# redhat-et/aws-k8s-ansible-provisioner

Measured on AMD Instinct MI355X. Metric: output tok/s + p50 TTFT, higher is better.
Workload: dtype bf16

## Files before the change

aws_k8s_ansible_provisioner_amd/csrc/kernels/kernels.h:

```cpp
#pragma once

#include <hip/hip_runtime.h>
#include <stdint.h>

#include "host_contract.h"

namespace akap {

void launch_rmsnorm(void* out, const void* x, const void* w, int rows, int d, int x_stride,
                    int out_stride, float eps, hipStream_t s);
void launch_fused_add_rmsnorm(void* out, void* residual, const void* x, const void* w, int rows,
                              int d, int x_stride, int out_stride, float eps, hipStream_t s);

void launch_qk_norm_rope_cache(const void* qkv, int qkv_stride, void* q_out, void* k_cache,
                               void* v_cache, const int64_t* positions, const int64_t* slots,
                               const float* cos_sin, const void* q_w, const void* k_w, int T,
                               int Hq, int Hkv, int D, int BS, float eps, int apply_rope,
                               hipStream_t s, int kv_fp8 = 0, int v_per_token = 0,
                               void* v_tail = nullptr, const int* tail_slot = nullptr,
                               int num_decode = 0, int q_rows = -1);
void launch_reshape_and_cache(const void* k, const void* v, void* k_cache, void* v_cache,
                              const int64_t* slots, int T, int Hkv, int D, int BS, hipStream_t s,
                              int kv_fp8 = 0);

// ... 131 lines not shown
void launch_moe_combine_split(const float* P, const float* wts, const int32_t* inv, void* out,
                              int T, int topk, int d, int S, int rows, hipStream_t s);

void launch_moe_topk_softmax(const void* logits, int ld, int E, int K, float* topk_w,
                             int32_t* topk_ids, int T, int renormalize, hipStream_t s);
void launch_moe_router_topk(const void* h, int ldh, const void* W, int d, int E, int K,
                            float* topk_w, int32_t* topk_ids, int T, int renormalize,
                            hipStream_t s);
void launch_moe_align(const int32_t* topk_ids, int n, int E, int block, int32_t* sorted_ids,
                      int32_t* expert_offsets, int32_t* num_padded, int32_t* inv,
                      int32_t* tile_expert, int max_tiles, hipStream_t s);
void launch_moe_gemm(const void* A, const void* W, void* Y, const int32_t* sorted_ids,
                     const int32_t* tile_expert, int max_tiles, int n_flat, int topk, int N,
                     int K, int lda, int gather, hipStream_t s);
void launch_moe_combine(const void* Y, const float* wts, const int32_t* inv, void* out, int T,
                        int topk, int d, hipStream_t s);

void launch_kv_gather(const void* cache, long plane_stride, int planes, int block_elems,
                      int cache_blocks, const int* block_ids, int nblk, void* out,
                      hipStream_t s);
void launch_kv_scatter(const void* in, void* cache, long plane_stride, int planes,
                       int block_elems, int cache_blocks, const int* block_ids, int nblk,
                       hipStream_t s);
struct KVPullArgs {
  const int64_t* src_planes;
  const int64_t* dst_planes;
  int planes, block_elems;
  const int* pairs;
  int nblk;
  __bf16* tail;
  const int* tail_jobs;
  int ntail, layers, tail_slots, Hkv, BS, D;
};
void launch_kv_pull(const KVPullArgs& a, hipStream_t s);

void launch_embedding_prep(const int64_t* ids, const void* table, const void* ln, void* residual,
                           void* a_out, float* ss_out, float* zbuf, long zn, int T, int d,
                           int vocab_start, int vocab_end, hipStream_t s);
void launch_embedding(const int64_t* ids, const void* table, void* out, int T, int d,
                      int vocab_start, int vocab_end, hipStream_t s);

struct CarArgs {
  __bf16* bufs[8];
  uint32_t* sigs[8];
  uint32_t* counter;
  uint32_t* err;
  int rank, world;
  size_t half_elems;
  int blocks;
};
struct CarEpi {
  __bf16* residual;
  const __bf16* ln;
  __bf16* aout;
  float* ss;
  int d;
};
void launch_custom_allreduce(const CarArgs& a, const void* in, void* out, long n, int two_shot,
                             hipStream_t s, const CarEpi* epi = nullptr);
size_t custom_allreduce_signal_bytes();
void launch_custom_allgather(const CarArgs& a, const void* in, void* out, long rows, int n,
                             hipStream_t s);
void launch_custom_broadcast(const CarArgs& a, void* buf, long bytes, int root, hipStream_t s);
void launch_custom_alltoall(const CarArgs& a, const void* in, void* out, long seg_elems,
                            hipStream_t s);
struct CarMulti {
  CarArgs args[8];
  const void* in[8];
  void* out[8];
  CarEpi epi[8];
  int use_epi;
  int warm;
};
void launch_custom_allreduce_multi(const CarMulti& m, int world, long n, int two_shot,
                                   hipStream_t s);

struct PrefetchList {
  const void* ptr[8];
  long bytes[8];
  int n;
};
void launch_l2_prefetch(const PrefetchList& L, uint32_t* sink, hipStream_t s);
void launch_h2d_stage(const void* host_src, void* dst, long bytes, hipStream_t s);

}
```

aws_k8s_ansible_provisioner_amd/csrc/kernels/prefetch.hip:

```cpp
#include "common.h"
#include "kernels.h"

namespace akap {

__global__ __launch_bounds__(256) void l2_prefetch_kernel(PrefetchList L, uint32_t* sink) {
  uint32_t acc = 0;
  const long gid = (long)blockIdx.x * 256 + threadIdx.x;
  const long stride = (long)gridDim.x * 256;
  for (int i = 0; i < L.n; ++i) {
    const u32x4* p = reinterpret_cast<const u32x4*>(L.ptr[i]);
    const long n16 = L.bytes[i] >> 4;
    for (long j = gid; j < n16; j += stride) acc ^= p[j].x;
  }
  if (acc == 0x9E3779B9u && gid == 0) sink[0] = acc;
}

void launch_l2_prefetch(const PrefetchList& L, uint32_t* sink, hipStream_t s) {
  long total = 0;
  for (int i = 0; i < L.n; ++i) total += L.bytes[i];
  if (total == 0) return;
  long blocks = (total / 16 + 255) / 256;
  if (blocks > 2048) blocks = 2048;
  l2_prefetch_kernel<<<(int)blocks, 256, 0, s>>>(L, sink);
}

__global__ __launch_bounds__(256) void h2d_stage_kernel(const uint8_t* __restrict__ src,
                                                        uint8_t* __restrict__ dst, long bytes) {
  const long gid = (long)blockIdx.x * 256 + threadIdx.x;
  const long stride = (long)gridDim.x * 256;
  const long n16 = bytes >> 4;
  for (long j = gid; j < n16; j += stride)
    reinterpret_cast<u32x4*>(dst)[j] = __builtin_nontemporal_load(reinterpret_cast<const u32x4*>(src) + j);
  for (long j = (n16 << 4) + gid; j < bytes; j += stride) dst[j] = src[j];
}

void launch_h2d_stage(const void* host_src, void* dst, long bytes, hipStream_t s) {
  if (bytes <= 0) return;
  long blocks = ((bytes >> 4) + 255) / 256;
  if (blocks < 1) blocks = 1;
  if (blocks > 64) blocks = 64;
  h2d_stage_kernel<<<(int)blocks, 256, 0, s>>>((const uint8_t*)host_src, (uint8_t*)dst, bytes);
}

}
```

aws_k8s_ansible_provisioner_amd/csrc/kernels/wgemm.hip:

```cpp
#include <cstdlib>

#include "gemm_common.h"

namespace akap {

constexpr int WNS = 3;

template <int WM>
struct WCfg {
  static constexpr int BM = 64 * WM;
  static constexpr int WN = 8 / WM;
  static constexpr int BN = WM == 4 ? 128 : 256;
  static constexpr int WC = BN / WN;
  static constexpr int JN = WC / 16;
  static constexpr int GA = WM;
  static constexpr int GW = BN / 64;
  static constexpr int G = GA + GW;
  static constexpr int SU = (BM + BN) * 8;
  static constexpr int EP = WC + 8;
};

template <int WM, bool NTW = false>
__global__ __launch_bounds__(512, 2) void wgemm_kernel(WGemmArgs p) {
  using C = WCfg<WM>;
// ... 117 lines not shown
  const bf16* X = static_cast<const bf16*>(p.X);
  const bf16* W = static_cast<const bf16*>(p.W);
  const int lr = lane >> 2;
  const int lc = (lane & 3) ^ ((0x1320 >> (4 * ((lr >> 2) & 3))) & 3);
  const bf16* asrc[GA];
  const bf16* wsrc[GW];
#pragma unroll
  for (int i = 0; i < GA; ++i) {
    const int row = (w * GA + i) * 16 + lr;
    asrc[i] = X + (size_t)(row < p.M ? row : 0) * p.ldx + lc * 8;
  }
#pragma unroll
  for (int i = 0; i < GW; ++i) {
    const int v = n0 + (w * GW + i) * 16 + lr;
    wsrc[i] = W + (size_t)(v < p.N ? v : 0) * p.ldw + lc * 8;
  }
  auto issue = [&](int step) {
    bf16x8* slot = lds + (step % NS) * SU;
    const int k0 = step * BK;
#pragma unroll
    for (int i = 0; i < GA; ++i) glds16(asrc[i] + k0, slot + (w * GA + i) * 64);
#pragma unroll
    for (int i = 0; i < GW; ++i)
      glds16<NTW ? kAuxNT : 0>(wsrc[i] + k0, slot + BM * 4 + (w * GW + i) * 64);
  };

  f32x4 acc[4][JN];
#pragma unroll
  for (int i = 0; i < 4; ++i)
#pragma unroll
    for (int j = 0; j < JN; ++j) acc[i][j] = f32x4{0.f, 0.f, 0.f, 0.f};

#pragma unroll
  for (int s = 0; s < NS - 1; ++s)
    if (s < nk) issue(s);
  for (int t = 0; t < nk; ++t) {
    if (t + 2 < nk) wait_vm<2 * G>();
    else if (t + 1 < nk) wait_vm<G>();
    else asm volatile("s_waitcnt vmcnt(0)" ::: "memory");
    asm volatile("s_waitcnt lgkmcnt(0)" ::: "memory");
    __builtin_amdgcn_s_barrier();
    if (t + NS - 1 < nk) issue(t + NS - 1);
    const bf16x8* slot = lds + (t % NS) * SU;
    bf16x8 af[4], bfr[JN];
#pragma unroll
    for (int i = 0; i < 4; ++i) af[i] = slot[ww_swz(wm * 64 + i * 16 + fr, fg)];
#pragma unroll
    for (int j = 0; j < JN; ++j) bfr[j] = slot[BM * 4 + ww_swz(wn * WC + j * 16 + fr, fg)];
#pragma unroll
    for (int i = 0; i < 4; ++i)
#pragma unroll
      for (int j = 0; j < JN; ++j)
        acc[i][j] = __builtin_amdgcn_mfma_f32_16x16x32_bf16(af[i], bfr[j], acc[i][j], 0, 0, 0);
  }

  asm volatile("s_waitcnt lgkmcnt(0)" ::: "memory");
  __builtin_amdgcn_s_barrier();
  bf16* et = reinterpret_cast<bf16*>(lds) + (size_t)w * 64 * EP;
#pragma unroll
  for (int i = 0; i < 4; ++i)
#pragma unroll
    for (int j = 0; j < JN; ++j)
#pragma unroll
      for (int r = 0; r < 4; ++r) et[(i * 16 + fg * 4 + r) * EP + j * 16 + fr] = f2bf(acc[i][j][r]);
  asm volatile("s_waitcnt lgkmcnt(0)" ::: "memory");
  bf16* Y = static_cast<bf16*>(p.Y);
  constexpr int CPR = WC / 8;
  for (int e = lane; e < 64 * CPR; e += 64) {
    const int rr = e / CPR, cc = e % CPR;
    const int row = wm * 64 + rr;
    const int col = n0 + wn * WC + cc * 8;
    if (row >= p.M || col >= p.N) continue;
    const bf16* src = et + rr * EP + cc * 8;
    bf16* dst = Y + (size_t)row * p.ldy + col;
    if (col + 8 <= p.N) {
      bf16x8 v;
#pragma unroll
      for (int q = 0; q < 8; ++q) v[q] = src[q];
      *reinterpret_cast<bf16x8*>(dst) = v;
    } else {
      for (int q = 0; q < p.N - col; ++q) dst[q] = src[q];
    }
  }
}

static int wgemm_wide() {
  static const int v = [] {
    const char* e = std::getenv("AKAP_WGEMM_WIDE");
    return e ? std::atoi(e) : 0;
  }();
  return v;
}

int wgemm_rows(int M) { return M <= 64 ? 1 : (M <= 128 ? 2 : 4); }

void launch_wgemm(const WGemmArgs& p, hipStream_t st) {
  if (p.M == 0 || p.N == 0) return;
  const int wmr = wgemm_rows(p.M);
  const int bm = 64 * wmr, bn = wmr == 4 ? 128 : 256;
  dim3 grid((p.N + bn - 1) / bn, (p.M + bm - 1) / bm);
  static const bool nt = [] {
    const char* e = std::getenv("AKAP_WGEMM_NT");
    return e == nullptr || std::atoi(e) != 0;
  }();
  if (wmr == 4 && p.M <= 256 && wgemm_wide() == 1 && p.K % 32 == 0) {
    const dim3 gw((p.N + 255) / 256);
    if (nt) wgemm_wide_kernel<true><<<gw, 512, 0, st>>>(p);
    else wgemm_wide_kernel<false><<<gw, 512, 0, st>>>(p);
    return;
  }
  switch (wmr) {
    case 1: if (nt) wgemm_kernel<1, true><<<grid, 512, 0, st>>>(p); else wgemm_kernel<1><<<grid, 512, 0, st>>>(p); break;
    case 2: if (nt) wgemm_kernel<2, true><<<grid, 512, 0, st>>>(p); else wgemm_kernel<2><<<grid, 512, 0, st>>>(p); break;
    default: if (nt) wgemm_kernel<4, true><<<grid, 512, 0, st>>>(p); else wgemm_kernel<4><<<grid, 512, 0, st>>>(p); break;
  }
}

}
```

aws_k8s_ansible_provisioner_amd/csrc/ops.cpp:

```cpp
#include <algorithm>
#include <cstdlib>
#include <cstring>
#include <vector>
#include <torch/library.h>
#include <ATen/ATen.h>
#include <c10/hip/HIPStream.h>

#include "kernels/kernels.h"
#include "op_args.h"


namespace {

using at::Tensor;
using akap::OpArgs, akap::kAlign16, akap::kContig, akap::kLastContig;

hipStream_t cur_stream() { return c10::hip::getCurrentHIPStream().stream(); }

OpArgs on_gpu(const char* op, const Tensor& t, const char* name) {
  TORCH_CHECK(t.defined() && t.is_cuda(), op, ": ", name, " must be a GPU tensor");
  return OpArgs(op, t.device());
}

void rmsnorm(Tensor out, Tensor x, Tensor w, double eps) {
// ... 604 lines not shown

void kv_scatter(Tensor buf, Tensor cache, Tensor block_ids) {
  const OpArgs a = on_gpu("kv_scatter", cache, "cache");
  const int planes = cache.size(0), nblk = block_ids.numel();
  akap::launch_kv_scatter(a.ptr(buf, "buf", {buf.scalar_type()},
                                (int64_t)planes * nblk * cache.stride(1)),
                          a.ptr(cache, "cache", {cache.scalar_type()}), cache.stride(0), planes,
                          cache.stride(1), cache.size(1), a.ptr<int>(block_ids, "block_ids"),
                          nblk, cur_stream());
}

void kv_pull(Tensor src_planes, Tensor dst_planes, int64_t block_elems, Tensor pairs,
             std::optional<Tensor> tail, std::optional<Tensor> tail_jobs, int64_t Hkv,
             int64_t BS, int64_t D) {
  const OpArgs o = on_gpu("kv_pull", dst_planes, "dst_planes");
  TORCH_CHECK(src_planes.numel() == dst_planes.numel() && src_planes.numel() % 2 == 0,
              "kv_pull: plane tables int64 [2L], same length");
  TORCH_CHECK(pairs.numel() % 2 == 0, "kv_pull: pairs [n, 2]");
  akap::KVPullArgs a{};
  a.src_planes = o.ptr<int64_t>(src_planes, "src_planes");
  a.dst_planes = o.ptr<int64_t>(dst_planes, "dst_planes");
  a.planes = src_planes.numel();
  a.block_elems = (int)block_elems;
  const bool byte_cache = (int64_t)a.block_elems * 2 == Hkv * BS * D;
  TORCH_CHECK(a.block_elems % 8 == 0 && (a.block_elems == Hkv * BS * D || byte_cache),
              "block = Hkv*BS*D (bf16) or Hkv*BS*D/2 (fp8 bytes viewed as bf16)");
  a.pairs = o.ptr<int>(pairs, "pairs");
  a.nblk = pairs.numel() / 2;
  a.Hkv = Hkv; a.BS = BS; a.D = D;
  a.layers = a.planes / 2;
  if (tail && tail_jobs && tail_jobs->numel()) {
    TORCH_CHECK(!byte_cache, "kv_pull: V-tail jobs need a bf16 cache");
    TORCH_CHECK(tail->dim() == 5 && tail->size(0) == a.layers && tail->size(2) == Hkv &&
                tail->size(3) == 8 && tail->size(4) == D, "kv_pull: tail [L, slots, Hkv, 8, D]");
    TORCH_CHECK(tail_jobs->numel() % 4 == 0, "kv_pull: tail_jobs [m, 4]");
    TORCH_CHECK(BS % 8 == 0, "kv_pull: block size % 8");
    a.tail = reinterpret_cast<__bf16*>(o.bf16(*tail, "tail"));
    a.tail_slots = tail->size(1);
    a.tail_jobs = o.ptr<int>(*tail_jobs, "tail_jobs");
    a.ntail = tail_jobs->numel() / 4;
  }
  akap::launch_kv_pull(a, cur_stream());
}

void pgemm(Tensor out, Tensor x, Tensor w, int64_t epi, std::optional<Tensor> offs) {
  const OpArgs o = on_gpu("pgemm", x, "x");
  TORCH_CHECK(x.dim() == 2 && out.dim() == 2, "pgemm: x, out must be 2-D");
  TORCH_CHECK(epi == akap::EPI_STORE || epi == akap::EPI_SILU, "pgemm: epilogue store | silu");
  akap::PGemmArgs a{};
  a.M = x.size(0);
  a.K = x.size(1);
  a.N = w.size(-2);
  TORCH_CHECK(w.size(-1) == a.K, "pgemm: w [.., N, K] must match x [M, K]");
  TORCH_CHECK(akap::pgemm_supported(a.M, a.N, a.K, x.stride(0)),
              "pgemm: N % 256 == 0 and K % 64 == 0 needed, X and each weight matrix below 2 GiB");
  TORCH_CHECK(out.size(0) == a.M && out.size(1) == (epi == akap::EPI_SILU ? a.N / 2 : a.N),
              "pgemm: out shape");
  TORCH_CHECK(w.dim() == (offs ? 3 : 2) && (!offs || offs->numel() == w.size(0)),
              "pgemm: w [N, K], or w [G, N, K] with offs [G]");
  a.offs = o.ptr<int>(offs, "offs");
  a.groups = offs ? offs->numel() : 0;
  a.X = o.bf16(x, "x", 0, kLastContig);
  a.W = o.bf16(w, "w");
  a.Y = o.bf16(out, "out", 0, kLastContig);
  a.ldx = x.stride(0);
  a.ldy = out.stride(0);
  TORCH_CHECK(a.ldx % 8 == 0 && a.ldy % 4 == 0,
              "pgemm: row strides must keep 16-B / 8-B alignment");
  akap::launch_pgemm(a, (int)epi, cur_stream());
}

void h2d_stage(Tensor dst, Tensor src) {
  const OpArgs a = on_gpu("h2d_stage", dst, "dst");
  TORCH_CHECK(src.defined() && !src.is_cuda() && src.is_pinned() && src.is_contiguous(),
              "h2d_stage: src must be contiguous pinned host memory");
  TORCH_CHECK(src.nbytes() == dst.nbytes(), "h2d_stage: size mismatch");
  void* dev_src = nullptr;
  TORCH_CHECK(hipHostGetDevicePointer(&dev_src, src.data_ptr(), 0) == hipSuccess,
              "h2d_stage: the pinned buffer has no device mapping");
  akap::launch_h2d_stage(dev_src, a.ptr(dst, "dst", {dst.scalar_type()}), (long)dst.nbytes(),
                         cur_stream());
}

void embedding(Tensor ids, Tensor table, Tensor out, int64_t vocab_start, int64_t vocab_end) {
  const OpArgs a = on_gpu("embedding", ids, "ids");
  TORCH_CHECK(table.dim() == 2 && table.size(1) % 8 == 0,
              "embedding: table [V, d] with d a multiple of 8");
  const int T = ids.numel(), d = table.size(1);
  akap::launch_embedding(a.ptr<int64_t>(ids, "ids"), a.bf16(table, "table"),
                         a.bf16(out, "out", (int64_t)T * d), T, d, vocab_start, vocab_end,
                         cur_stream());
}

void embedding_prep(Tensor ids, Tensor table, Tensor ln, Tensor residual, Tensor a_out,
                    Tensor ss_out, Tensor zbuf, int64_t vocab_start, int64_t vocab_end) {
  const OpArgs a = on_gpu("embedding_prep", ids, "ids");
  TORCH_CHECK(table.dim() == 2, "embedding_prep: table [V, d]");
  const int T = ids.numel(), d = table.size(1);
  TORCH_CHECK(d % 8 == 0 && ln.numel() == d,
              "embedding_prep: embedding dim multiple of 8, ln of length d");
  TORCH_CHECK(residual.numel() == (int64_t)T * d && a_out.numel() == (int64_t)T * d,
              "embedding_prep: residual / a_out [T, d]");
  akap::launch_embedding_prep(a.ptr<int64_t>(ids, "ids"), a.bf16(table, "table"),
                              a.bf16(ln, "ln"), a.bf16(residual, "residual"),
                              a.bf16(a_out, "a_out"), a.ptr<float>(ss_out, "ss_out", T),
                              a.ptr<float>(zbuf, "zbuf"), zbuf.numel(), T, d, vocab_start,
                              vocab_end, cur_stream());
}

}


namespace {
struct CarComm {
  int device = 0;
  akap::CarArgs args{};
  void* buf = nullptr;
  void* sig = nullptr;
  std::vector<void*> opened;
};
std::vector<CarComm*>& car_table() {
  static std::vector<CarComm*> t;
  return t;
}
CarComm* car_get(int64_t h) {
  auto& t = car_table();
  TORCH_CHECK(h >= 0 && h < (int64_t)t.size() && t[h] != nullptr, "bad custom all-reduce handle");
  return t[h];
}
#define HIP_OK(x)                                                                     \
  do {                                                                                \
    hipError_t e_ = (x);                                                              \
    TORCH_CHECK(e_ == hipSuccess, #x " failed: ", hipGetErrorString(e_));             \
  } while (0)
}

int64_t car_create(int64_t device, int64_t rank, int64_t world, int64_t max_elems,
                   int64_t blocks) {
  TORCH_CHECK(world >= 1 && world <= 8 && rank >= 0 && rank < world, "world must be 1..8");
  TORCH_CHECK(blocks >= 1 && blocks <= 128, "car blocks must be 1..128");
  TORCH_CHECK(max_elems % 8 == 0, "max_elems % 8");
  const c10::DeviceGuard g(c10::Device(c10::DeviceType::CUDA, (int)device));
  auto* c = new CarComm();
  c->device = (int)device;
  const size_t buf_bytes = (size_t)4 * max_elems * sizeof(uint16_t);
  const size_t sig_bytes = akap::custom_allreduce_signal_bytes();
  HIP_OK(hipExtMallocWithFlags(&c->buf, buf_bytes, hipDeviceMallocUncached));
  HIP_OK(hipExtMallocWithFlags(&c->sig, sig_bytes, hipDeviceMallocUncached));
  HIP_OK(hipMemset(c->sig, 0, sig_bytes));
  void* local = nullptr;
  HIP_OK(hipMalloc(&local, 4096));
  HIP_OK(hipMemset(local, 0, 4096));
  HIP_OK(hipDeviceSynchronize());
  c->args.counter = reinterpret_cast<uint32_t*>(local);
  c->args.err = reinterpret_cast<uint32_t*>(local) + 1023;
  c->args.rank = (int)rank;
  c->args.world = (int)world;
  c->args.half_elems = (size_t)max_elems;
  c->args.blocks = (int)blocks;
  for (int p = 0; p < 8; ++p) { c->args.bufs[p] = nullptr; c->args.sigs[p] = nullptr; }
  c->args.bufs[rank] = reinterpret_cast<__bf16*>(c->buf);
  c->args.sigs[rank] = reinterpret_cast<uint32_t*>(c->sig);
  car_table().push_back(c);
  return (int64_t)car_table().size() - 1;
}

// ... 225 lines not shown

void car_destroy(int64_t h) {
  CarComm* c = car_get(h);
  const c10::DeviceGuard g(c10::Device(c10::DeviceType::CUDA, c->device));
  (void)hipDeviceSynchronize();
  for (void* p : c->opened) (void)hipIpcCloseMemHandle(p);
  (void)hipFree(c->buf);
  (void)hipFree(c->sig);
  (void)hipFree(c->args.counter);
  delete c;
  car_table()[h] = nullptr;
}

TORCH_LIBRARY(akap, m) {
  m.def("rmsnorm(Tensor(a!) out, Tensor x, Tensor w, float eps) -> ()");
  m.def("fused_add_rmsnorm(Tensor(a!) out, Tensor(b!) residual, Tensor x, Tensor w, float eps) -> ()");
  m.def(
      "qk_norm_rope_cache(Tensor qkv, Tensor(a!) q_out, Tensor(b!) k_cache, Tensor(c!) v_cache, "
      "Tensor positions, Tensor slots, Tensor cos_sin, Tensor? q_w, Tensor? k_w, int Hq, int Hkv, "
      "float eps, bool apply_rope, bool decode=False, Tensor(d!)? v_tail=None, "
      "Tensor? tail_slot=None, int num_decode=0, int q_rows=-1) -> ()");
  m.def("reshape_and_cache(Tensor k, Tensor v, Tensor(a!) k_cache, Tensor(b!) v_cache, Tensor slots) -> ()");
  m.def("silu_and_mul(Tensor(a!) out, Tensor x) -> ()");
  m.def(
      "paged_attention_prefill(Tensor(a!) out, Tensor q, Tensor k_cache, Tensor v_cache, "
      "Tensor block_tables, Tensor seq_lens, Tensor q_start, Tensor tile_seq, Tensor tile_row, "
      "int G, float scale, int tile_rows=128) -> ()");
  m.def(
      "paged_attention_prefill_qprep(Tensor(a!) out, Tensor qkv, Tensor k_cache, Tensor v_cache, "
      "Tensor block_tables, Tensor seq_lens, Tensor q_start, Tensor tile_seq, Tensor tile_row, "
      "Tensor positions, Tensor cos_sin, Tensor? q_w, int G, float scale, float eps, "
      "int tile_rows=128) -> ()");
  m.def(
      "paged_attention_decode(Tensor(a!) out, Tensor q, Tensor k_cache, Tensor v_cache, "
      "Tensor block_tables, Tensor seq_lens, Tensor? q_start, Tensor(b!) part_m, Tensor(c!) part_l, "
      "Tensor(d!) part_o, int num_parts, int part_size, int G, float scale, "
      "Tensor? v_tail=None, Tensor? tail_slot=None) -> ()");
  m.def(
      "paged_attention_decode_fused(Tensor(a!) out, Tensor qkv, Tensor(b!) k_cache, "
      "Tensor(c!) v_cache, Tensor block_tables, Tensor seq_lens, Tensor positions, Tensor slots, "
      "Tensor cos_sin, Tensor? q_w, Tensor? k_w, Tensor(d!) part_m, Tensor(e!) part_l, "
      "Tensor(f!) part_o, int num_parts, int part_size, int G, float scale, float eps, "
      "Tensor(g!)? v_tail=None, Tensor? tail_slot=None) -> ()");
  m.def(
      "sample(Tensor logits, Tensor temperature, Tensor top_k, Tensor top_p, Tensor seeds, "
      "Tensor steps, Tensor(a!) out_tokens, Tensor(b!) out_logprobs, "
      "bool greedy_logprobs, Tensor(c!) ws, Tensor(d!) tickets, bool filtered=True) -> ()");
  m.def(
      "apply_penalties(Tensor(a!) logits, Tensor rows, Tensor toks, Tensor counts, "
      "Tensor presence, Tensor frequency, Tensor repetition) -> ()");
  m.def("argmax(Tensor logits, Tensor(a!) out) -> ()");
  m.def(
      "gemm(Tensor(a!) out, Tensor x, Tensor w, Tensor(b!) ws, int splitk, "
      "Tensor(c!)? counters=None) -> ()");
  m.def("gemm_splitk(int M, int N, int K) -> int");
  m.def(
      "dgemm(Tensor(a!) out, Tensor x, Tensor w, Tensor(b!) ws, int pro, int splitk, int pf, "
      "Tensor? r=None, Tensor(c!)? rout=None, Tensor? ln=None, float eps=1e-6, int epi=0, "
      "Tensor? ss_in=None, Tensor(d!)? ss_out=None, Tensor(e!)? aout=None, "
      "Tensor? ln_out=None, int bn=0, int ns=0, Tensor(f!)? counters=None, int bm=64) -> ()");
  m.def("wgemm(Tensor(a!) out, Tensor x, Tensor w) -> ()");
  m.def("qgemm(Tensor(a!) out, Tensor x, Tensor wq, Tensor scale) -> ()");
  m.def("dequant_fp8(Tensor(a!) out, Tensor wq, Tensor scale) -> ()");
  m.def("pgemm(Tensor(a!) out, Tensor x, Tensor w, int epi=0, Tensor? offs=None) -> ()");
  m.def("kgemm(Tensor(a!) out, Tensor x, Tensor w, int bm, int epi, float eps, Tensor? ss_in, "
        "Tensor(b!)? ss_out, Tensor(c!)? aout, Tensor? ln_out) -> ()");
  m.def("l2_prefetch(Tensor[] ts, Tensor(a!) sink) -> ()");
  m.def("car_create(int device, int rank, int world, int max_elems, int blocks=128) -> int");
  m.def("car_ipc_handles(int h) -> Tensor");
  m.def("car_open(int h, Tensor handles) -> ()");
  m.def("car_all_reduce(int h, Tensor inp, Tensor(a!) out, bool two_shot) -> ()");
  m.def("car_error(int h) -> int");
  m.def("car_error_word(int h) -> Tensor");
  m.def("car_link_local(int h, int[] peers) -> ()");
  m.def("car_all_reduce_multi(int[] hs, Tensor[] ins, Tensor(a!)[] outs, bool two_shot, "
        "Tensor(b!)[]? epi=None, bool warm=False) -> ()");
  m.def("car_all_reduce_resnorm(int h, Tensor inp, Tensor(a!) residual, Tensor ln, "
        "Tensor(b!) aout, Tensor(c!) ss, bool two_shot) -> ()");
  m.def("car_destroy(int h) -> ()");
  m.def("car_all_gather(int h, Tensor inp, Tensor(a!) out) -> ()");
  m.def("car_broadcast(int h, Tensor(a!) buf, int root) -> ()");
  m.def("car_all_to_all(int h, Tensor inp, Tensor(a!) out) -> ()");
  m.def("h2d_stage(Tensor(a!) dst, Tensor src) -> ()");
  m.def("ipc_export(Tensor t) -> Tensor");
  m.def("ipc_open(Tensor blob, int device) -> int");
  m.def("ipc_close(int addr) -> ()");
  m.def(
      "kv_pull(Tensor src_planes, Tensor dst_planes, int block_elems, Tensor pairs, "
      "Tensor(a!)? tail, Tensor? tail_jobs, int Hkv, int BS, int D) -> ()");
  m.def("moe_topk_softmax(Tensor logits, Tensor(a!) topk_w, Tensor(b!) topk_ids, bool renorm) -> ()");
  m.def("moe_router_topk(Tensor h, Tensor router, Tensor(a!) topk_w, Tensor(b!) topk_ids, bool renorm) -> ()");
  m.def(
      "moe_align(Tensor topk_ids, int E, int block, Tensor(a!) sorted_ids, Tensor(b!) offsets, "
      "Tensor(c!) num_padded, Tensor(d!) inv, Tensor(e!) tile_expert) -> ()");
  m.def(
      "moe_gemm(Tensor(a!) out, Tensor a, Tensor w, Tensor sorted_ids, Tensor tile_expert, "
      "int n_flat, int topk, bool gather) -> ()");
  m.def("moe_combine(Tensor y, Tensor wts, Tensor inv, Tensor(a!) out) -> ()");
  m.def(
      "moe_dgemm(Tensor(a!) out, Tensor a, Tensor w, Tensor sorted_ids, Tensor tile_expert, "
      "int n_flat, int topk, bool gather, bool silu, int pf, int bm=32, int splitk=1) -> ()");
  m.def(
      "moe_combine_split(Tensor partials, Tensor wts, Tensor inv, Tensor(a!) out, int splitk, "
      "int rows) -> ()");
  m.def("kv_gather(Tensor cache, Tensor block_ids, Tensor(a!) out) -> ()");
  m.def("kv_scatter(Tensor buf, Tensor(a!) cache, Tensor block_ids) -> ()");
  m.def("embedding(Tensor ids, Tensor table, Tensor(a!) out, int vocab_start, int vocab_end) -> ()");
  m.def("embedding_prep(Tensor ids, Tensor table, Tensor ln, Tensor(a!) residual, "
        "Tensor(b!) a_out, Tensor(c!) ss_out, Tensor(d!) zbuf, int vocab_start, "
        "int vocab_end) -> ()");
}

TORCH_LIBRARY_IMPL(akap, CompositeExplicitAutograd, m) {
  m.impl("gemm_splitk", &gemm_splitk);
  m.impl("car_create", &car_create);
  m.impl("car_ipc_handles", &car_ipc_handles);
  m.impl("car_open", &car_open);
  m.impl("car_error", &car_error);
  m.impl("car_error_word", &car_error_word);
  m.impl("car_link_local", &car_link_local);
  m.impl("car_destroy", &car_destroy);
  m.impl("ipc_open", &ipc_open);
  m.impl("ipc_close", &ipc_close);
  m.impl("h2d_stage", &h2d_stage);
}

TORCH_LIBRARY_IMPL(akap, CUDA, m) {
  m.impl("rmsnorm", &rmsnorm);
  m.impl("fused_add_rmsnorm", &fused_add_rmsnorm);
  m.impl("qk_norm_rope_cache", &qk_norm_rope_cache);
  m.impl("reshape_and_cache", &reshape_and_cache);
  m.impl("silu_and_mul", &silu_and_mul);
  m.impl("paged_attention_prefill", &paged_attention_prefill);
  m.impl("paged_attention_prefill_qprep", &paged_attention_prefill_qprep);
  m.impl("paged_attention_decode", &paged_attention_decode);
  m.impl("paged_attention_decode_fused", &paged_attention_decode_fused);
  m.impl("sample", &sample);
  m.impl("apply_penalties", &apply_penalties);
  m.impl("argmax", &argmax);
  m.impl("gemm", &gemm);
  m.impl("dgemm", &dgemm);
  m.impl("wgemm", &wgemm);
  m.impl("qgemm", &qgemm);
  m.impl("dequant_fp8", &dequant_fp8);
  m.impl("pgemm", &pgemm);
  m.impl("kgemm", &kgemm);
  m.impl("moe_topk_softmax", &moe_topk_softmax);
  m.impl("moe_router_topk", &moe_router_topk);
  m.impl("moe_align", &moe_align);
  m.impl("moe_gemm", &moe_gemm);
  m.impl("moe_combine", &moe_combine);
  m.impl("moe_dgemm", &moe_dgemm);
  m.impl("moe_combine_split", &moe_combine_split);
  m.impl("car_all_reduce", &car_all_reduce);
  m.impl("l2_prefetch", &l2_prefetch);
  m.impl("car_all_reduce_multi", &car_all_reduce_multi);
  m.impl("car_all_reduce_resnorm", &car_all_reduce_resnorm);
  m.impl("kv_gather", &kv_gather);
  m.impl("kv_scatter", &kv_scatter);
  m.impl("kv_pull", &kv_pull);
  m.impl("car_all_gather", &car_all_gather);
  m.impl("car_broadcast", &car_broadcast);
  m.impl("car_all_to_all", &car_all_to_all);
  m.impl("ipc_export", &ipc_export);
  m.impl("embedding", &embedding);
  m.impl("embedding_prep", &embedding_prep);
}
```

aws_k8s_ansible_provisioner_amd/engine/model_runner.py:

```python
from __future__ import annotations

import math
import os
import time
from typing import Optional

import numpy as np
import torch

from ..utils import profiling
from .. import ops
from ..models import moe as moe_mod
from ..models.config import ModelConfig
from ..models.transformer import AttnBatch, DecoderLM
from ..parallel.state import ParallelState, drain_pending_collectives, get_state
from .config import EngineConfig

H2D_KERNEL = os.environ.get("AKAP_H2D_KERNEL", "1") != "0"

DEFAULT_BUCKETS = [1, 2, 4, 8, 16, 24, 32, 48, 64, 80, 96, 112, 128, 160, 192, 224, 256, 320,
                   384, 448, 512]


DECODE_FIELDS = ("input_ids", "positions", "slots", "seeds", "seq_lens", "temperature", "top_p",
# ... 98 lines not shown
            return
        g0, cnt = n & ~7, n % 8
        blk, grp = int(block_table[g0 // self.bs]), (g0 % self.bs) // 8
        if self.is_gpu:
            planes = self.kv_planes()
            ops.kv_pull(ops.plane_table(planes), self.num_blocks, planes, [], self.model.hkv,
                        self.bs, self.model.D, tail=self._tail, tail_jobs=[(blk, grp, cnt, slot)])
            return
        for vt, vc in zip(self.v_tails, self.v_caches):
            vt[slot, :, :cnt].copy_(vc[blk, :, grp, :, :cnt].transpose(-1, -2))

    def kv_planes(self) -> list:
        out = []
        for seg in self.kv_segs:
            kv = seg.view(torch.bfloat16) if seg.dtype == torch.uint8 else seg
            L, two, NB, be = kv.shape
            out.append(kv.view(L * two, NB, be))
        return out

    def _derive_num_blocks(self) -> int:
        elem = 1 if self.ecfg.kv_cache_dtype.startswith("fp8") else 2
        per_block = self.mcfg.num_layers * 2 * self.model.hkv * self.bs * self.model.D * elem
        if not self.is_gpu:
            return max(64, min(4096, (self.max_seqs * self.ecfg.max_model_len) // self.bs + 8))
        torch.cuda.synchronize()
        free, total = torch.cuda.mem_get_info(self.device)
        used = torch.cuda.memory_reserved(self.device) + 2**30
        d = self.mcfg.hidden_size
        width = d * 4 + (self.model.hq + 2 * self.model.hkv) * self.model.D + 3 * self.model.ffn
        act = self.cap_tokens * width * 2 * 3 + self.max_seqs * self.mcfg.vocab_size * 12
        reserve = act + 3 * 2**30
        budget = min(total * self.ecfg.gpu_memory_utilization - used, free) - reserve
        n = int(budget // per_block)
        if self.ecfg.kv_cache_max_gib:
            n = min(n, int(self.ecfg.kv_cache_max_gib * 2**30 // per_block))
        if n < self.max_blocks:
            raise RuntimeError(f"not enough HBM for the KV cache ({budget / 2**30:.1f} GiB)")
        return n

    def _pinned(self, n, dtype):
        t = torch.zeros(n, dtype=dtype, pin_memory=self.is_gpu)
        return t

    def _alloc_buffers(self) -> None:
        S, T, TL, mb = self.max_seqs, self.cap_tokens, self.cap_tiles, self.max_blocks
        spec = {
            "input_ids": (T, torch.int64), "positions": (T, torch.int64), "slots": (T, torch.int64),
            "seq_lens": (S, torch.int32), "q_start": (S + 1, torch.int32),
            "block_tables": (S * mb, torch.int32), "tile_seq": (TL, torch.int32),
            "tile_row": (TL, torch.int32), "logits_idx": (S, torch.int64),
            "req_ids": (S, torch.int64), "sample_mask": (S, torch.int32),
            "temperature": (S, torch.float32), "top_p": (S, torch.float32),
            "top_k": (S, torch.int32), "seeds": (S, torch.int64), "steps": (S, torch.int32),
            "src_rows": (S, torch.int64),
            "tail_slot": (T, torch.int32),
        }
        self.h = {k: self._pinned(n, dt) for k, (n, dt) in spec.items()}
        self.np = {k: v.numpy() for k, v in self.h.items()}
        self.d = {k: torch.zeros(n, dtype=dt, device=self.device) for k, (n, dt) in spec.items()
                  if k not in ("req_ids", "sample_mask")}
        self.d_bt = self.d["block_tables"].view(S, mb)
        fields = [(k, self.h[k].dtype, S) for k in DECODE_FIELDS] + [("block_tables", torch.int32,
                                                                      S * mb)]
        off, lay = 0, {}
        for k, dt, n in fields:
            lay[k] = (off, dt, n)
            off += -(-n * torch.empty(0, dtype=dt).element_size() // 16) * 16
        self.hdecs = [self._pinned(off, torch.uint8) for _ in range(2)]
        self.ddec = torch.zeros(off, dtype=torch.uint8, device=self.device)
        view = lambda buf, o, dt, n: buf[o:o + n * torch.empty(0, dtype=dt).element_size()].view(dt)
        self.hd_nps = [{k: view(h, o, dt, n).numpy() for k, (o, dt, n) in lay.items()}
                       for h in self.hdecs]
        self._dslot = 0
        self.dd = {k: view(self.ddec, o, dt, n) for k, (o, dt, n) in lay.items()}
        self._h2d_kernel = False
        if self.is_gpu and H2D_KERNEL:
            try:
                torch.ops.akap.h2d_stage(self.ddec[:16], self.hdecs[0][:16])
                self._h2d_kernel = True
            except RuntimeError as e:
                self.log(f"[runner] staging kernel unavailable ({e}); using hipMemcpyAsync")
        self.dd_bt = self.dd["block_tables"].view(S, mb)
        self._dec_bt_off = lay["block_tables"][0]
        self.out_tokens = torch.zeros(S, dtype=torch.int64, device=self.device)
        self.tok_host = [self._pinned(S, torch.int64) for _ in range(2)]
        self._err_host = [self._pinned(1, torch.int32) for _ in range(7)]
        self._pending_err = None
        self._follower_err: list = []
        self._follower_slot = 0
        self._replays = 0
        self.out_logprobs = torch.zeros(S, dtype=torch.float32, device=self.device)
        self.workspace = ops.decode_workspace(S, self.model.hkv, self.G, self.num_parts,
                                              self.device)

    def host_buffers(self) -> dict:
        return self.np

    def _stage_decode(self, n: int) -> int:
        slot = self._dslot
        self._dslot ^= 1
        hd_np = self.hd_nps[slot]
        for k in DECODE_FIELDS:
            hd_np[k][:n] = self.np[k][:n]
        nb = n * self.max_blocks
        hd_np["block_tables"][:nb] = self.np["block_tables"][:nb]
        end = self._dec_bt_off + nb * 4
        if self._h2d_kernel:
            torch.ops.akap.h2d_stage(self.ddec[:end], self.hdecs[slot][:end])
        else:
            self.ddec[:end].copy_(self.hdecs[slot][:end], non_blocking=True)
        return slot

    def _h2d(self, key: str, n: int) -> torch.Tensor:
        dst = self.d[key][:n]
        dst.copy_(self.h[key][:n], non_blocking=True)
        return dst

    def _sample(self, logits: torch.Tensor, n: int, extras: Optional[dict] = None,
                src: Optional[dict] = None):
        lp = False
        if extras:
            pen = extras.get("penalties")
            if pen is not None:
                dev = logits.device
                rows, toks, counts, pres, freq, rep = pen
                ops.apply_penalties(
                    logits, torch.from_numpy(rows).to(dev), torch.from_numpy(toks).to(dev),
                    torch.from_numpy(counts).to(dev), torch.from_numpy(pres).to(dev),
                    torch.from_numpy(freq).to(dev), torch.from_numpy(rep).to(dev))
            lp = bool(extras.get("logprobs"))
        d = self.d if src is None else src
        ntop = int(extras.get("top_logprobs") or 0) if extras else 0
        if ntop > 0:
            t = d["temperature"][:n].float()
            x = logits.float() / torch.where(t > 0, t, torch.ones_like(t))[:, None]
            vals, idx = torch.topk(x, min(ntop, x.shape[-1]), dim=-1)
            vals = vals - torch.logsumexp(x, dim=-1, keepdim=True)
            self.last_top = (idx.cpu().numpy(), vals.cpu().numpy())
        mode = self._sample_mode(n)
        return ops.sample(logits, d["temperature"][:n], d["top_k"][:n],
                          d["top_p"][:n], d["seeds"][:n], d["steps"][:n],
                          out_tokens=self.out_tokens[:n], out_logprobs=self.out_logprobs[:n],
                          greedy_logprobs=lp, filtered=mode == "filtered",
                          greedy_only=mode == "greedy" and not lp)

    def _sample_mode(self, n: int) -> str:
        if self._capture_mode is not None:
            return self._capture_mode
        if not self.is_gpu or self._peer_step:
            return "filtered"
        npd, V = self.np, self.mcfg.vocab_size
        t, k, p = npd["temperature"][:n], npd["top_k"][:n], npd["top_p"][:n]
        if not (t > 0).any():
            return "greedy"
        if ((t > 0) & (((k > 0) & (k < V)) | ((p > 0) & (p < 1)))).any():
            return "filtered"
        return "plain"

    def _graph_for(self, n: int, B: int):
        g = self.graphs.get(n)
        if g is None or self._peer_step:
            return g
        mode = self._sample_mode(B)
        return g if mode == "plain" else self.graphs_v[(mode, n)]

    PREFILL_FIELDS = ("input_ids", "positions", "slots", "seq_lens", "q_start", "block_tables",
                      "tile_seq", "tile_row", "logits_idx", "temperature", "top_p", "top_k",
                      "seeds", "steps", "tail_slot")

    def _prefill_extents(self, info: dict) -> dict:
        T, B, nt, ns = info["num_tokens"], info["num_seqs"], info["num_tiles"], info["num_samples"]
        return {"input_ids": T, "positions": T, "slots": T, "seq_lens": B, "q_start": B + 1,
                "block_tables": B * self.max_blocks, "tile_seq": nt, "tile_row": nt,
                "logits_idx": ns, "temperature": ns, "top_p": ns, "top_k": ns, "seeds": ns,
                "steps": ns, "tail_slot": T}

    def _stage_prefill(self, info: dict) -> dict:
        ext = self._prefill_extents(info)
        lay, off = {}, 0
        for k in self.PREFILL_FIELDS:
            nb = ext[k] * self.h[k].element_size()
            lay[k] = (off, ext[k])
            off += -(-nb // 16) * 16
        end = off
        if self._hpre is None or self._hpre.numel() < end:
            cap = max(end, 1 << 16)
            self._hpre = self._pinned(cap, torch.uint8)
            self._dpre = torch.zeros(cap, dtype=torch.uint8, device=self.device)
        tp = self._tp_bcast_inputs
        if not (tp and self.ps.tp_rank != 0):
            hb = self._hpre.numpy()
            for k in self.PREFILL_FIELDS:
                o, n = lay[k]
# ... 97 lines not shown
    def _check_err(h) -> None:
        if h is not None and int(h[0]) != 0:
            from ..parallel.comm import CollectiveTimeout

            raise CollectiveTimeout(
                "custom IPC collective timed out in a decode step (a peer rank stalled): the "
                "step's tokens are discarded and the engine is marked unhealthy")

    def _check_follower_err(self) -> None:
        pend = self._follower_err
        while pend and pend[0][0].query():
            ev, h = pend.pop(0)
            self._check_err(h)

    @property
    def _ep_moe(self) -> bool:
        return self.ps.world_size > 1 and any(
            getattr(getattr(layer, "moe", None), "mode", None) == "ep"
            for layer in getattr(self.model, "layers", []))

    def _ep_overflowed(self) -> bool:
        return self._ep_moe and int(moe_mod.MoEBlock.overflow_flag(self.device).item()) != 0

    def _pad_host(self, B: int, n: int) -> None:
        if n <= B:
            return
        npd = self.np
        npd["input_ids"][B:n] = 0
        npd["positions"][B:n] = 0
        npd["slots"][B:n] = -1
        npd["seq_lens"][B:n] = 0
        npd["temperature"][B:n] = 0.0
        npd["top_p"][B:n] = 1.0
        npd["top_k"][B:n] = 0
        npd["seeds"][B:n] = 0
        npd["steps"][B:n] = 0
        npd["src_rows"][B:n] = 0
        npd["tail_slot"][B:n] = -1

    def execute_decode(self, info: dict) -> torch.Tensor:
        B = info["num_seqs"]
        n = B
        graph = None
        if self.graphs:
            for b in self.buckets:
                if b >= B:
                    n, graph = b, self.graphs[b]
                    break
        if not (self._tp_bcast_inputs and self.ps.tp_rank != 0):
            self._pad_host(B, n)
            self._stage_decode(n)
        extras = info.get("extras")
        if graph is not None and not extras:
            if not (self._tp_bcast_inputs and self.ps.tp_rank != 0):
                graph = self._graph_for(n, B)
            graph.replay()
        else:
            self._decode_body(n, extras)
        self._ep_rerun_if_overflowed(n, extras)
        if self.ps.world_size > 1:
            from ..parallel import comm

            comm.check_deferred()
        self._pending_err = self._err_probe(2)
        return self.out_tokens[:B]

    def _ep_rerun_if_overflowed(self, n: int, extras: Optional[dict]) -> None:
        if self._ep_overflowed():
            self.ep_overflow_steps += 1
            with moe_mod.exact_dispatch():
                self._decode_body(n, extras)

    def launch_decode(self, info: dict, chained: bool = False):
        B = info["num_seqs"]
        n, graph = B, None
        for b in self.buckets:
            if b >= B:
                n, graph = b, self.graphs[b]
                break
        if graph is None and self.is_gpu:
            raise RuntimeError(f"no decode graph holds {B} rows")
        self._pad_host(B, n)
        with profiling.phase("akap.decode"):
            slot = self._stage_decode(n)
            if chained:
                torch.index_select(self.out_tokens[:self.max_seqs], 0, self.dd["src_rows"][:n],
                                   out=self.dd["input_ids"][:n])
            if graph is not None:
                self._graph_for(n, B).replay()
            else:
                self._decode_body(n)
        if not self.is_gpu:
            return None, self.out_tokens[:B].clone(), self._err_probe(slot)
        host = self.tok_host[slot][:B]
        host.copy_(self.out_tokens[:B], non_blocking=True)
        err = self._err_probe(slot)
        ev = torch.cuda.Event()
        ev.record()
        return ev, host, err

    def replay_decode(self, info: dict) -> None:
        B = info["num_seqs"]
        n, graph = B, None
        for b in self.buckets:
            if b >= B:
                n, graph = b, self.graphs[b]
                break
        self._replays += 1
        if graph is not None:
            if self._replays != _FAULT_SKIP_REPLAY:
                graph.replay()
        else:
            self._decode_body(n)
        if self.is_gpu and self.ps.car is not None:
            self._check_follower_err()
            slot = self._follower_slot = (self._follower_slot + 1) % 4
            h = self._err_probe(3 + slot)
            if h is not None:
                ev = torch.cuda.Event()
                ev.record()
                self._follower_err.append((ev, h))

    def _bucket(self, B: int) -> int:
        for b in self.buckets:
            if b >= B:
                return b
        return B

    def execute_decode_eager(self, info: dict) -> None:
        n = self._bucket(info["num_seqs"])
        self._decode_body(n)
        self._ep_rerun_if_overflowed(n, None)

    @classmethod
    def wait_decode(cls, handle) -> np.ndarray:
        ev, host, err = handle
        if ev is not None:
            ev.synchronize()
        cls._check_err(err)
        return host.numpy()

    def execute(self, info: dict) -> np.ndarray:
        if info["is_prefill"]:
            with profiling.phase("akap.prefill"):
                toks = self.execute_prefill(info)
        else:
            with profiling.phase("akap.decode"):
                toks = self.execute_decode(info)
        if info["is_prefill"]:
            self._pending_err = self._err_probe(2)
        extras = info.get("extras")
        if extras and extras.get("logprobs"):
            self.last_logprobs = self.out_logprobs[:toks.shape[0]].to("cpu").numpy()
        out = toks.to("cpu").numpy()
        err, self._pending_err = self._pending_err, None
        self._check_err(err)
        return out

    def _graph_has_collectives(self) -> bool:
        if self.ps.world_size > 1:
            return True
        return any(getattr(getattr(layer, "moe", None), "mode", None) == "ep"
                   for layer in getattr(self.model, "layers", []))

    def capture_graphs(self) -> None:
        maxbs = min(self.ecfg.cuda_graph_max_bs or self.max_seqs, self.max_seqs)
        self.buckets = [b for b in DEFAULT_BUCKETS if b <= maxbs]
        if not self.buckets or self.buckets[-1] < maxbs:
            self.buckets.append(maxbs)
        t0 = time.time()
# ... 70 lines not shown
```

Measured before the change: 51250.

## Fuse decode staging with chained token gather; add persistent wgemm for small M

Adds a decode_stage kernel that copies the pinned host staging buffer to the device and, in the same launch, gathers the previous step's output tokens into input_ids. This replaces a separate index_select launch and so removes one launch per decode step. Separately, it adds a persistent wgemm kernel for M<=256 with the 4-row config. Each CU loops over N tiles with a 3-slot LDS pipeline that carries prefetch across tile boundaries. This new GEMM path is on by default and brings correctness and register-pressure risk.

```diff
diff --git a/aws_k8s_ansible_provisioner_amd/csrc/kernels/kernels.h b/aws_k8s_ansible_provisioner_amd/csrc/kernels/kernels.h
--- a/aws_k8s_ansible_provisioner_amd/csrc/kernels/kernels.h
+++ b/aws_k8s_ansible_provisioner_amd/csrc/kernels/kernels.h
@@ -237,5 +237,7 @@
 };
 void launch_l2_prefetch(const PrefetchList& L, uint32_t* sink, hipStream_t s);
 void launch_h2d_stage(const void* host_src, void* dst, long bytes, hipStream_t s);
+void launch_decode_stage(const void* host_src, void* dst, long bytes, long rows_off, int64_t* ids,
+                         const int64_t* out_tokens, int n, int n_tok, hipStream_t s);
 
 }
diff --git a/aws_k8s_ansible_provisioner_amd/csrc/kernels/prefetch.hip b/aws_k8s_ansible_provisioner_amd/csrc/kernels/prefetch.hip
--- a/aws_k8s_ansible_provisioner_amd/csrc/kernels/prefetch.hip
+++ b/aws_k8s_ansible_provisioner_amd/csrc/kernels/prefetch.hip
@@ -42,4 +42,43 @@
   h2d_stage_kernel<<<(int)blocks, 256, 0, s>>>((const uint8_t*)host_src, (uint8_t*)dst, bytes);
 }
 
+__global__ __launch_bounds__(256) void decode_stage_kernel(const uint8_t* __restrict__ src,
+                                                           uint8_t* __restrict__ dst, long bytes,
+                                                           long rows_off, int64_t* ids,
+                                                           const int64_t* __restrict__ out_tokens,
+                                                           int n, int n_tok) {
+  const long gid = (long)blockIdx.x * 256 + threadIdx.x;
+  const long stride = (long)gridDim.x * 256;
+  const long n16 = bytes >> 4;
+  const long lo = reinterpret_cast<const uint8_t*>(ids) - dst, hi = lo + (long)n * 8;
+  for (long j = gid; j < n16; j += stride) {
+    const u32x4 v = __builtin_nontemporal_load(reinterpret_cast<const u32x4*>(src) + j);
+    const long b = j << 4;
+    if (b + 16 <= lo || b >= hi) {
+      reinterpret_cast<u32x4*>(dst)[j] = v;
+    } else {
+      uint2* d = reinterpret_cast<uint2*>(dst + b);
+      if (b < lo || b >= hi) d[0] = uint2{v.x, v.y};
+      if (b + 8 < lo || b + 8 >= hi) d[1] = uint2{v.z, v.w};
+    }
+  }
+  for (long j = (n16 << 4) + gid; j < bytes; j += stride)
+    if (j < lo || j >= hi) dst[j] = src[j];
+  const int64_t* rows = reinterpret_cast<const int64_t*>(src + rows_off);
+  for (long i = gid; i < n; i += stride) {
+    const int64_t r = rows[i];
+    ids[i] = (r >= 0 && r < n_tok) ? out_tokens[r] : 0;
+  }
 }
+
+void launch_decode_stage(const void* host_src, void* dst, long bytes, long rows_off, int64_t* ids,
+                         const int64_t* out_tokens, int n, int n_tok, hipStream_t s) {
+  if (bytes <= 0) return;
+  long blocks = ((bytes >> 4) + 255) / 256;
+  if (blocks < 1) blocks = 1;
+  if (blocks > 64) blocks = 64;
+  decode_stage_kernel<<<(int)blocks, 256, 0, s>>>((const uint8_t*)host_src, (uint8_t*)dst, bytes,
+                                                  rows_off, ids, out_tokens, n, n_tok);
+}
+
+}
diff --git a/aws_k8s_ansible_provisioner_amd/csrc/kernels/wgemm.hip b/aws_k8s_ansible_provisioner_amd/csrc/kernels/wgemm.hip
--- a/aws_k8s_ansible_provisioner_amd/csrc/kernels/wgemm.hip
+++ b/aws_k8s_ansible_provisioner_amd/csrc/kernels/wgemm.hip
@@ -223,6 +223,154 @@
       for (int q = 0; q < p.N - col; ++q) dst[q] = src[q];
     }
   }
+}
+
+template <bool NTW>
+__global__ __launch_bounds__(512, 2) void wgemm_persist_kernel(WGemmArgs p, int tiles) {
+  using C = WCfg<4>;
+  constexpr int NS = WNS, JN = C::JN;
+  constexpr int EH = 32 * C::EP;
+  static_assert(NS == 3 && 4 * EH * 2 <= C::SU * 16, "four waves' epilogue passes fit one slot");
+  __shared__ bf16x8 lds[NS * C::SU];
+
+  const int nk = p.K / WBK;
+  const int tid = threadIdx.x, lane = tid & 63, w = tid >> 6;
+  const int wm = w / C::WN, wn = w % C::WN;
+  const int fr = lane & 15, fg = lane >> 4;
+  const bf16* X = static_cast<const bf16*>(p.X);
+  const bf16* W = static_cast<const bf16*>(p.W);
+  bf16* Y = static_cast<bf16*>(p.Y);
+  const int lr = lane >> 3, lc = (lane & 7) ^ (lane >> 3);
+  const bf16* asrc[C::GA];
+  const bf16* wsrc[C::GW];
+#pragma unroll
+  for (int i = 0; i < C::GA; ++i) {
+    const int row = (w * C::GA + i) * 8 + lr;
+    asrc[i] = X + (size_t)(row < p.M ? row : 0) * p.ldx + lc * 8;
+  }
+  auto wrows = [&](int tile) {
+#pragma unroll
+    for (int i = 0; i < C::GW; ++i) {
+      const int v = tile * C::BN + (w * C::GW + i) * 8 + lr;
+      wsrc[i] = W + (size_t)(v < p.N ? v : 0) * p.ldw + lc * 8;
+    }
+  };
+
+  const int total = (tiles - (int)blockIdx.x + (int)gridDim.x - 1) / (int)gridDim.x * nk;
+  int issued = 0, ik = 0, islot = 0, itile = blockIdx.x;
+  wrows(itile);
+  auto issue_next = [&]() {
+    bf16x8* slot = lds + islot * C::SU;
+    const int k0 = ik * WBK;
+#pragma unroll
+    for (int i = 0; i < C::GA; ++i) glds16(asrc[i] + k0, slot + (w * C::GA + i) * 64);
+#pragma unroll
+    for (int i = 0; i < C::GW; ++i)
+      glds16<NTW ? kAuxNT : 0>(wsrc[i] + k0, slot + C::BM * 8 + (w * C::GW + i) * 64);
+    ++issued;
+    islot = islot == NS - 1 ? 0 : islot + 1;
+    if (++ik == nk) {
+      ik = 0;
+      itile += gridDim.x;
+      if (issued < total) wrows(itile);
+    }
+  };
+
+  issue_next();
+  if (issued < total) issue_next();
+  int cslot = 0, g = 0;
+  for (int tile = blockIdx.x; tile < tiles; tile += gridDim.x) {
+    f32x4 acc[4][JN];
+#pragma unroll
+    for (int i = 0; i < 4; ++i)
+#pragma unroll
+      for (int j = 0; j < JN; ++j) acc[i][j] = f32x4{0.f, 0.f, 0.f, 0.f};
+    for (int kk = 0; kk < nk; ++kk, ++g) {
+      if (g + 1 < total) wait_vm<C::G>();
+      else asm volatile("s_waitcnt vmcnt(0)" ::: "memory");
+      asm volatile("s_waitcnt lgkmcnt(0)" ::: "memory");
+      __builtin_amdgcn_s_barrier();
+      if (kk != nk - 1 && issued < total) issue_next();
+      const bf16x8* slot = lds + cslot * C::SU;
+#pragma unroll
+      for (int ks = 0; ks < 2; ++ks) {
+        bf16x8 af[4], bfr[JN];
+#pragma unroll
+        for (int i = 0; i < 4; ++i) af[i] = slot[swz8(wm * 64 + i * 16 + fr, ks * 4 + fg)];
+#pragma unroll
+        for (int j = 0; j < JN; ++j)
+          bfr[j] = slot[C::BM * 8 + swz8(wn * C::WC + j * 16 + fr, ks * 4 + fg)];
+#pragma unroll
+        for (int i = 0; i < 4; ++i)
+#pragma unroll
+          for (int j = 0; j < JN; ++j)
+            acc[i][j] = __builtin_amdgcn_mfma_f32_16x16x32_bf16(af[i], bfr[j], acc[i][j], 0, 0, 0);
+      }
+      cslot = cslot == NS - 1 ? 0 : cslot + 1;
+    }
+    const int rslot = cslot == 0 ? NS - 1 : cslot - 1;
+    const int pslot = cslot == NS - 1 ? 0 : cslot + 1;
+
+    asm volatile("s_waitcnt lgkmcnt(0)" ::: "memory");
+    __builtin_amdgcn_s_barrier();
+    bf16* et = reinterpret_cast<bf16*>(lds + (w < 4 ? rslot : pslot) * C::SU) + (w & 3) * EH;
+    int el = lane;
+    asm volatile("" : "+v"(el));
+    const int er = el >> 3, ec = (el & 7) * 8;
+    const int col = tile * C::BN + wn * C::WC + ec;
+    bf16* ecol = Y + (size_t)(wm * 64 + er) * p.ldy + col;
+    bf16* ew = et + ((el >> 4) * 4) * C::EP + (el & 15);
+#pragma unroll
+    for (int h = 0; h < 2; ++h) {
+#pragma unroll
+      for (int i = 0; i < 2; ++i)
+#pragma unroll
+        for (int j = 0; j < JN; ++j)
+#pragma unroll
+          for (int r = 0; r < 4; ++r)
+            ew[(i * 16 + r) * C::EP + j * 16] = f2bf(acc[h * 2 + i][j][r]);
+      asm volatile("s_waitcnt lgkmcnt(0)" ::: "memory");
+#pragma unroll
+      for (int s = 0; s < 4; ++s) {
+        const int rr = h * 32 + s * 8;
+        if (wm * 64 + rr + er >= p.M || col >= p.N) continue;
+        const bf16* src = et + (s * 8 + er) * C::EP + ec;
+        bf16* dst = ecol + (size_t)rr * p.ldy;
+        if (col + 8 <= p.N) {
+          bf16x8 v;
+#pragma unroll
+          for (int q = 0; q < 8; ++q) v[q] = src[q];
+          *reinterpret_cast<bf16x8*>(dst) = v;
+        } else {
+          for (int q = 0; q < p.N - col; ++q) dst[q] = src[q];
+        }
+      }
+      asm volatile("s_waitcnt lgkmcnt(0)" ::: "memory");
+    }
+    if (issued < total) {
+      __builtin_amdgcn_s_barrier();
+      issue_next();
+    }
+  }
+}
+
+static int wgemm_cus() {
+  static const int v = [] {
+    int dev = 0, n = 0;
+    if (hipGetDevice(&dev) != hipSuccess ||
+        hipDeviceGetAttribute(&n, hipDeviceAttributeMultiprocessorCount, dev) != hipSuccess || n <= 0)
+      n = 256;
+    return n;
+  }();
+  return v;
+}
+
+static int wgemm_body() {
+  static const int v = [] {
+    const char* e = std::getenv("AKAP_WGEMM_BODY");
+    return e ? std::atoi(e) : 1;
+  }();
+  return v;
 }
 
 static int wgemm_wide() {
@@ -250,6 +398,13 @@
     else wgemm_wide_kernel<false><<<gw, 512, 0, st>>>(p);
     return;
   }
+  if (wmr == 4 && p.M <= 256 && wgemm_body() != 0) {
+    const int tiles = (p.N + 127) / 128, cus = wgemm_cus();
+    const dim3 gp(tiles > cus ? cus : tiles);
+    if (nt) wgemm_persist_kernel<true><<<gp, 512, 0, st>>>(p, tiles);
+    else wgemm_persist_kernel<false><<<gp, 512, 0, st>>>(p, tiles);
+    return;
+  }
   switch (wmr) {
     case 1: if (nt) wgemm_kernel<1, true><<<grid, 512, 0, st>>>(p); else wgemm_kernel<1><<<grid, 512, 0, st>>>(p); break;
     case 2: if (nt) wgemm_kernel<2, true><<<grid, 512, 0, st>>>(p); else wgemm_kernel<2><<<grid, 512, 0, st>>>(p); break;
diff --git a/aws_k8s_ansible_provisioner_amd/csrc/ops.cpp b/aws_k8s_ansible_provisioner_amd/csrc/ops.cpp
--- a/aws_k8s_ansible_provisioner_amd/csrc/ops.cpp
+++ b/aws_k8s_ansible_provisioner_amd/csrc/ops.cpp
@@ -710,6 +710,37 @@
                          cur_stream());
 }
 
+void decode_stage(Tensor dst, Tensor src, Tensor input_ids, Tensor out_tokens, int64_t rows_off,
+                  int64_t n, bool chained) {
+  const OpArgs a = on_gpu("decode_stage", dst, "dst");
+  TORCH_CHECK(src.defined() && !src.is_cuda() && src.is_pinned(),
+              "decode_stage: src must be pinned host memory");
+  const OpArgs host("decode_stage", src.device());
+  void* host_src = host.ptr(src, "src", {src.scalar_type()}, 0, kContig | kAlign16);
+  const int64_t bytes = dst.nbytes();
+  TORCH_CHECK((int64_t)src.nbytes() == bytes, "decode_stage: size mismatch");
+  void* dev_src = nullptr;
+  TORCH_CHECK(hipHostGetDevicePointer(&dev_src, host_src, 0) == hipSuccess,
+              "decode_stage: the pinned buffer has no device mapping");
+  char* d = static_cast<char*>(a.ptr(dst, "dst", {dst.scalar_type()}, 0, kContig | kAlign16));
+  if (!chained) {
+    akap::launch_h2d_stage(dev_src, d, (long)bytes, cur_stream());
+    return;
+  }
+  TORCH_CHECK(n >= 0 && rows_off >= 0 && rows_off % 8 == 0 && rows_off + n * 8 <= bytes,
+              "decode_stage: src_rows [", rows_off, ", +", n, " int64) must lie in the ", bytes,
+              " staged bytes");
+  int64_t* ids = a.ptr<int64_t>(input_ids, "input_ids", n);
+  const int64_t* toks = a.ptr<int64_t>(out_tokens, "out_tokens", 1);
+  const char* t = reinterpret_cast<const char*>(toks);
+  TORCH_CHECK(t + out_tokens.nbytes() <= d || t >= d + bytes,
+              "decode_stage: out_tokens must not overlap dst");
+  TORCH_CHECK(t + out_tokens.nbytes() <= (const char*)ids || t >= (const char*)(ids + n),
+              "decode_stage: out_tokens must not overlap input_ids");
+  akap::launch_decode_stage(dev_src, d, (long)bytes, (long)rows_off, ids, toks, (int)n,
+                            (int)out_tokens.numel(), cur_stream());
+}
+
 void embedding(Tensor ids, Tensor table, Tensor out, int64_t vocab_start, int64_t vocab_end) {
   const OpArgs a = on_gpu("embedding", ids, "ids");
   TORCH_CHECK(table.dim() == 2 && table.size(1) % 8 == 0,
@@ -1101,6 +1132,8 @@
   m.def("car_broadcast(int h, Tensor(a!) buf, int root) -> ()");
   m.def("car_all_to_all(int h, Tensor inp, Tensor(a!) out) -> ()");
   m.def("h2d_stage(Tensor(a!) dst, Tensor src) -> ()");
+  m.def("decode_stage(Tensor(a!) dst, Tensor src, Tensor(b!) input_ids, Tensor out_tokens, "
+        "int rows_off, int n, bool chained) -> ()");
   m.def("ipc_export(Tensor t) -> Tensor");
   m.def("ipc_open(Tensor blob, int device) -> int");
   m.def("ipc_close(int addr) -> ()");
@@ -1142,6 +1175,7 @@
   m.impl("ipc_open", &ipc_open);
   m.impl("ipc_close", &ipc_close);
   m.impl("h2d_stage", &h2d_stage);
+  m.impl("decode_stage", &decode_stage);
 }
 
 TORCH_LIBRARY_IMPL(akap, CUDA, m) {
diff --git a/aws_k8s_ansible_provisioner_amd/engine/model_runner.py b/aws_k8s_ansible_provisioner_amd/engine/model_runner.py
--- a/aws_k8s_ansible_provisioner_amd/engine/model_runner.py
+++ b/aws_k8s_ansible_provisioner_amd/engine/model_runner.py
@@ -204,6 +204,7 @@
                 self.log(f"[runner] staging kernel unavailable ({e}); using hipMemcpyAsync")
         self.dd_bt = self.dd["block_tables"].view(S, mb)
         self._dec_bt_off = lay["block_tables"][0]
+        self._dec_rows_off = lay["src_rows"][0]
         self.out_tokens = torch.zeros(S, dtype=torch.int64, device=self.device)
         self.tok_host = [self._pinned(S, torch.int64) for _ in range(2)]
         self._err_host = [self._pinned(1, torch.int32) for _ in range(7)]
@@ -218,7 +219,7 @@
     def host_buffers(self) -> dict:
         return self.np
 
-    def _stage_decode(self, n: int) -> int:
+    def _stage_decode(self, n: int, chained: bool = False) -> int:
         slot = self._dslot
         self._dslot ^= 1
         hd_np = self.hd_nps[slot]
@@ -228,9 +229,14 @@
         hd_np["block_tables"][:nb] = self.np["block_tables"][:nb]
         end = self._dec_bt_off + nb * 4
         if self._h2d_kernel:
-            torch.ops.akap.h2d_stage(self.ddec[:end], self.hdecs[slot][:end])
+            torch.ops.akap.decode_stage(self.ddec[:end], self.hdecs[slot][:end],
+                                        self.dd["input_ids"], self.out_tokens,
+                                        self._dec_rows_off, n, chained)
         else:
             self.ddec[:end].copy_(self.hdecs[slot][:end], non_blocking=True)
+            if chained:
+                torch.index_select(self.out_tokens[:self.max_seqs], 0, self.dd["src_rows"][:n],
+                                   out=self.dd["input_ids"][:n])
         return slot
 
     def _h2d(self, key: str, n: int) -> torch.Tensor:
@@ -494,10 +500,7 @@
             raise RuntimeError(f"no decode graph holds {B} rows")
         self._pad_host(B, n)
         with profiling.phase("akap.decode"):
-            slot = self._stage_decode(n)
-            if chained:
-                torch.index_select(self.out_tokens[:self.max_seqs], 0, self.dd["src_rows"][:n],
-                                   out=self.dd["input_ids"][:n])
+            slot = self._stage_decode(n, chained)
             if graph is not None:
                 self._graph_for(n, B).replay()
             else:
```

Measured after the change: 50990. No clear change (-0.5%).
